# RaghuvirJonnagiri/LatticeBoltzmannSimulations

Hardware: AMD Instinct MI355X
Metric: MLUPS (million lattice updates/sec) D2Q9 MRT cavity (higher is better)
Workload: dtype f32

## Files before the change

### latticeboltzmannsimulations_amd/csrc/lbm_plan.hip

```cpp
#include "lbm_host.hpp"

namespace lbmhost {

bool frame_lds_fits(const Plan& pl, int S, bool deep_rows, int extra, long long budget) {
    if (!pl.frame_lds) return false;
    const int F = pl.tb_f, L = pl.frame_seg, m = S - 1, np = pl.semantics == LBM_SEM_BOUNCE_BACK_SOLID ? Q : pl.nplanes;
    const long long row_strip = (long long)(L + 2 * m + 2) * (F + m + (deep_rows ? m + extra : 0) + 2);
    const long long col_strip = (long long)(F + m + 2) * (L + 2 * m + extra + 2);
    return 2 * np * std::max(row_strip, col_strip) * pl.es <= budget;
}
int pairs_waves(int S) { return std::min(SP_MAX_WAVES, S + 2); }
StreamPlan plan_stream_on(const Plan& pl, int S, int ncu, long long* cost_out) {
    const bool walls = walls_inside(pl);
    const int V = 16 / pl.es, Rr = stream_rim(S, V), TXu = 64 * V - 2 * Rr, F = walls ? 0 : pl.tb_f;
    const int cols = pl.geo.nx - 2 * F;
    const int rows = walls ? pl.geo.ny - pl.tb_f * neighbours(pl) : pl.geo.ny - 2 * F;
    StreamPlan best{walls ? stream_walls_strips(pl.geo.nx, S, V) : (cols + TXu - 1) / TXu, 1, rows};
    long long best_cost = -1;
    for (int n = 1; n <= 256 && n * 8 <= std::max(rows, 8); ++n) {
        const int H = (rows + n - 1) / n, nseg = (rows + H - 1) / H;
        const long long segs = (long long)best.nstrips * nseg, rounds = (segs + ncu - 1) / ncu;
        long long iters = H + 2 * (S - 1) + ST_WAVES - 1;
        if (pl.kern == Kern::stream_pairs) {
            const long long Wv = pairs_waves(S), np = (H + 2 * (S - 1) + 1) / 2;
            iters = 2 * Wv * ((np + Wv - 1) / Wv) + 2 * Wv;
        }
        const long long cost = rounds * iters;
        if (best_cost < 0 || cost < best_cost) { best_cost = cost; best.nsegy = nseg; best.H = H; }
    }
    if (cost_out) *cost_out = best_cost;
    return best;
}
StreamPlan plan_stream(const Plan& pl, int S) {
    long long cost0 = 0;
    const StreamPlan p0 = plan_stream_on(pl, S, pl.ncu, &cost0);
    const bool walls = walls_inside(pl);
    if (!(is_slab(pl) && pl.deep_halo && (pl.frame_fused || walls) && pl.edge_reserve) || S < 3) return p0;
    if ((long long)p0.nstrips * p0.nsegy > pl.ncu) return p0;
    const int nb = neighbours(pl), L = pl.frame_seg;
    const long long n_edge = walls ? (long long)nb * p0.nstrips
                                   : (long long)nb * p0.nstrips + 2LL * frame_segs(pl.geo.ny, L) + (2LL - nb) * frame_segs(pl.geo.nx, L);
    const long long edge_it = pl.tb_f + 2 * (S - 1) + ST_WAVES - 1;
    if (walls ? cost0 > 3 * edge_it : 4 * cost0 > 7 * edge_it) return p0;
    StreamPlan best = p0;
    long long best_cost = cost0 + edge_it * ((n_edge + pl.ncu - 1) / pl.ncu);
    const long long grain = walls ? 32 : 1;
    auto in_grains = [&](long long n) { return (n + grain - 1) / grain * grain; };
    if (walls && in_grains((long long)p0.nstrips * p0.nsegy) + in_grains(n_edge) <= pl.ncu) best_cost = std::max(cost0, edge_it);
    for (int div = 1; div <= (walls ? 1 : 3); ++div) {
        const long long r = in_grains((n_edge + div - 1) / div);
        if (r < 1 || r > pl.ncu / 2) continue;
        long long cb = 0;
        const StreamPlan sp = plan_stream_on(pl, S, pl.ncu - (int)r, &cb);
        const long long cost = std::max(cb, edge_it * ((n_edge + r - 1) / r));
        if (cost < best_cost) { best_cost = cost; best = sp; }
    }
    return best;
}

bool lag_replayable(const Plan& pl, int S) {
    if (S <= 1) return true;
    if (!pl.lazy_lag || pl.push) return false;
    if (!is_slab(pl)) return true;
    return pl.deep_halo && S - 1 >= 3;
}

int unit_steps(const Plan& pl, int left, bool raw, bool own_transport) {
    if (left < 1) return 0;
    if (pl.kern == Kern::none || raw) return 1;
    const int T = pl.tb_steps;
    if (is_slab(pl) && !pl.deep_halo && !own_transport) return 1;
    if (!lag_replayable(pl, T)) {
        if (left >= T + 1) return T;
        if (T >= 3 && left - 1 >= 3) return left - 1;
        return 1;
    }
    if (T == 2) return left >= 2 ? 2 : 1;
    const int m = is_slab(pl) ? 4 : 3;
    if (left >= T) {
        const int r = left - T;
        if (r == 0 || r >= m) return T;
        if (left - m >= m) return left - m;
        return T;
    }
    return left >= m ? left : 1;
}

Route unit_route(const Plan& pl, int S, bool replay) {
    const bool slab = is_slab(pl), deep = slab && pl.deep_halo;
    if (replay && S < 3) return Route::single_steps;
    if (!slab && ((walls_inside(pl) && S >= 2) || (S >= 3 && pl.frame_fused && (replay || !(pl.kern == Kern::stream && pl.frame_beside)))))
        return Route::one_launch;
    if (S >= 3 && deep && streaming(pl) && (pl.frame_fused || walls_inside(pl))) return Route::edges_bulk;
    if (S >= 3 && pl.frame_fused && (!slab || deep)) return Route::fused_frame;
    return Route::frame_passes;
}


std::string validate_params(const lbm_params* p) {
    if (!p || p->struct_size != (int32_t)sizeof(lbm_params)) return std::string("lbm_params.struct_size mismatch");
    if (p->nx < 4 || p->ny < 4) return std::string("nx, ny must be >= 4");
    if (p->y0 < 0 || p->ny_local < 2 || p->y0 + p->ny_local > p->ny) return std::string("slab rows out of range (ny_local >= 2)");
    if (p->ny_local > 65535) return std::string("ny_local > 65535 not supported");
    if (p->dtype != LBM_F32 && p->dtype != LBM_F64) return std::string("dtype must be LBM_F32 or LBM_F64");
    if (p->collision < LBM_SRT || p->collision > LBM_MRT) return std::string("collision must be SRT, TRT or MRT");
    if (p->semantics < LBM_SEM_MRT_PY || p->semantics > LBM_SEM_BOUNCE_BACK_SOLID) return std::string("bad semantics");
    if (p->turb != 0 && p->turb != 1) return std::string("turb must be 0 or 1");
    if (p->turb == 1 && p->semantics != LBM_SEM_MRT_GPU) return std::string("turb = 1 (Smagorinsky, MRT_GPU.py:368-387) exists only with MRT_GPU semantics");
    if (p->kernel < LBM_KERNEL_AUTO || p->kernel > LBM_KERNEL_STREAM) return std::string("bad kernel variant");
    if (p->kernel == LBM_KERNEL_PUSH && (p->turb || p->batch > 1 || p->y0 != 0 || p->ny_local != p->ny))
        return std::string("kernel = PUSH (the reference's two-launch scheme, for A/B) takes one whole lattice without the closure");
    if (p->layout < LBM_LAYOUT_AUTO || p->layout > LBM_LAYOUT_ROWS) return std::string("bad layout");
    if (p->batch < 0 || p->batch > 65535) return std::string("batch must be 0 .. 65535");
    if (p->arith != LBM_ARITH_STRICT && p->arith != LBM_ARITH_FAST && p->arith != LBM_ARITH_PROMOTED)
        return std::string("arith must be LBM_ARITH_STRICT, LBM_ARITH_FAST or LBM_ARITH_PROMOTED");
    if (p->arith == LBM_ARITH_PROMOTED && p->semantics != LBM_SEM_MRT_GPU)
        return std::string("arith = promoted exists only with MRT_GPU semantics (promotion is a property of MRT_GPU.py's CUDA text; "
                           "MRT.py semantics is NumPy fp64)");
    if (p->arith == LBM_ARITH_PROMOTED && (p->flags & LBM_FLAG_STREAM_PAIRS))
        return std::string("arith = promoted does not run on the streaming kernel with two rows per wave (LBM_FLAG_STREAM_PAIRS)");
    if ((p->flags & LBM_FLAG_SOLID_TILES) && p->semantics != LBM_SEM_BOUNCE_BACK_SOLID)
        return std::string("LBM_FLAG_SOLID_TILES (solid obstacles on the multi-step tile kernel) needs a solid mask: semantics = LBM_SEM_BOUNCE_BACK_SOLID");
    if (p->semantics == LBM_SEM_BOUNCE_BACK_SOLID) {
        if (p->y0 != 0 || p->ny_local != p->ny)
            return std::string("solid obstacles (LBM_SEM_BOUNCE_BACK_SOLID) take whole lattices: no slabs (y0 = 0, ny_local = ny)");
        if (p->flags & LBM_FLAG_SOLID_TILES) {
            if (p->kernel != LBM_KERNEL_AUTO && p->kernel != LBM_KERNEL_TB)
                return std::string("LBM_FLAG_SOLID_TILES runs the tile kernel, kernel = AUTO or TB: STREAM / VEC / PUSH have no solid path, GENERIC is "
                                   "one step per launch (leave the flag out)");
            if (p->tb_steps == 2)
                return std::string("LBM_FLAG_SOLID_TILES: tb_steps must be 0 (default) or 3 .. 5 (the two-step tile kernel has no solid path)");
        } else if (p->kernel != LBM_KERNEL_AUTO && p->kernel != LBM_KERNEL_GENERIC)
            return std::string("solid obstacles (LBM_SEM_BOUNCE_BACK_SOLID) step one step per launch, kernel = AUTO or GENERIC: TB / STREAM / VEC / PUSH "
                               "never compute a cell next to a solid one (the tile kernel does with LBM_FLAG_SOLID_TILES)");
    }
    if (p->semantics == LBM_SEM_BOUNCE_BACK || p->semantics == LBM_SEM_BOUNCE_BACK_SOLID) {
        if (p->arith == LBM_ARITH_PROMOTED)
            return std::string("arith = promoted (MRT_GPU.py's CUDA text) does not exist with bounce-back walls (LBM_SEM_BOUNCE_BACK)");
        if (p->kernel == LBM_KERNEL_PUSH || p->kernel == LBM_KERNEL_VEC)
            return std::string("kernel = PUSH / VEC have MRT_GPU.py's wall rules built in: bounce-back walls (LBM_SEM_BOUNCE_BACK) run GENERIC, TB or STREAM");
        if (p->flags & (LBM_FLAG_STREAM_WALLS | LBM_FLAG_STREAM_PAIRS))
            return std::string("LBM_FLAG_STREAM_WALLS / STREAM_PAIRS: the streaming kernels with the walls inside have MRT_GPU.py's wall rules built in, "
                               "bounce-back walls (LBM_SEM_BOUNCE_BACK) run with the wall frame");
    }
    if (p->batch > 1 && (p->y0 != 0 || p->ny_local != p->ny)) return std::string("a batch of lattices cannot be slab-decomposed");
    if (p->ny_local_min < 0 || p->ny_local_min > p->ny_local) return std::string("ny_local_min must be 0 or the smallest ny_local of all ranks (<= ny_local)");
    if (p->tb_steps != 0 && (p->tb_steps < 2 || p->tb_steps > SP_MAX_S)) return std::string("tb_steps must be 0 (default) or 2 .. " + std::to_string(SP_MAX_S));
    if (p->frame_seg != 0 && p->frame_seg < 8) return std::string("frame_seg must be 0 (default) or >= 8");
    if ((p->flags & LBM_FLAG_NT_ON) && (p->flags & LBM_FLAG_NT_OFF)) return std::string("LBM_FLAG_NT_ON and LBM_FLAG_NT_OFF exclude each other");
    return std::string();
}

static int ny_plan(const lbm_params& p) { return p.ny_local_min > 0 ? p.ny_local_min : p.ny_local; }
static bool one_launch(const Plan& pl) { return pl.batch == 1 && !is_slab(pl) && pl.frame_fused; }

struct Forced {
    int nt = 0, frame_beside = 0;
    bool stream_walls = false, stream_pairs = false, no_stream_walls = false, no_tail_tiles = false;
};
static Forced decode_flags(const lbm_params& p, Plan& pl) {
    const auto on = [&](int bit) { return (p.flags & bit) != 0; };
    pl.deep_halo = p.semantics == LBM_SEM_MRT_GPU && !on(LBM_FLAG_NO_DEEP_HALO);
    pl.frame_fused = !on(LBM_FLAG_FRAME_UNFUSED);
    pl.frame_lds = !on(LBM_FLAG_NO_FRAME_LDS);
    pl.frame_wide = !on(LBM_FLAG_FRAME_NARROW);
    pl.lazy_lag = !on(LBM_FLAG_EAGER_LAG);
    pl.xcd_bands = !on(LBM_FLAG_NO_XCD_BANDS);
    pl.edge_first = !on(LBM_FLAG_NO_EDGE_FIRST);
    pl.edge_reserve = !on(LBM_FLAG_NO_EDGE_RESERVE);
    pl.comm_priority = !on(LBM_FLAG_COMM_PRIORITY_OFF);
    Forced f;
    f.nt = on(LBM_FLAG_NT_ON) ? 1 : on(LBM_FLAG_NT_OFF) ? -1 : 0;
    f.frame_beside = on(LBM_FLAG_FRAME_BESIDE_ON) ? 1 : on(LBM_FLAG_FRAME_BESIDE_OFF) ? -1 : 0;
    f.stream_walls = on(LBM_FLAG_STREAM_WALLS);
    f.stream_pairs = on(LBM_FLAG_STREAM_PAIRS);
    f.no_stream_walls = on(LBM_FLAG_NO_STREAM_WALLS);
    f.no_tail_tiles = on(LBM_FLAG_NO_TAIL_TILES);
    pl.solid_tiles = on(LBM_FLAG_SOLID_TILES);
    return f;
}

static void plan_geometry(Plan& pl, const lbm_params& p, const Forced& f) {
    pl.es = p.dtype == LBM_F32 ? 4 : 8;
    pl.geo.nx = p.nx;
    pl.geo.ny = p.ny_local;
    pl.geo.y0 = p.y0;
    pl.geo.NY = p.ny;
    pl.geo.pitch = ((p.nx + 2 * GH) + 3) / 4 * 4;
    pl.nplanes = p.turb ? Q + 2 : Q;
    if (p.semantics == LBM_SEM_BOUNCE_BACK_SOLID) pl.nplanes = Q + 1;
    pl.semantics = p.semantics;
    if (p.layout == LBM_LAYOUT_PLANES) {
        pl.geo.plane = (long long)pl.geo.pitch * (p.ny_local + 2 * GHY);
        pl.geo.row = pl.geo.pitch;
    } else {
        pl.geo.plane = pl.geo.pitch;
        pl.geo.row = (long long)pl.nplanes * pl.geo.pitch;
    }
    pl.batch = p.batch > 1 ? p.batch : 1;
    pl.bstride = (long long)pl.nplanes * pl.geo.pitch * (p.ny_local + 2 * GHY);
    pl.lat_bytes = (size_t)pl.bstride * pl.batch * pl.es;
    pl.use_nt = f.nt ? f.nt > 0 : pl.lat_bytes > ((size_t)192 << 20);
}

static std::string plan_kernel(Plan& pl, const lbm_params& p, const Forced& f, bool device) {
    const int nyp = ny_plan(p), V = 16 / pl.es;
    const bool slab = is_slab(pl);
    if (p.semantics == LBM_SEM_BOUNCE_BACK_SOLID) {
        pl.use_vec = p.nx % V == 0 && p.kernel != LBM_KERNEL_GENERIC;
        pl.kern = Kern::none;
        if (!pl.solid_tiles) return std::string();
        if (p.nx % V != 0 || p.nx < 32 || nyp < 32)
            return "LBM_FLAG_SOLID_TILES needs what kernel = TB needs: nx % (16 / sizeof(real)) == 0, nx >= 32 and ny >= 32";
        pl.kern = Kern::tile;
        return std::string();
    }
    const bool can_vec = p.semantics == LBM_SEM_MRT_GPU && p.nx % V == 0;
    if (p.kernel == LBM_KERNEL_VEC && !can_vec) return "kernel = VEC needs MRT_GPU semantics and nx % (16 / sizeof(real)) == 0";
    pl.push = p.kernel == LBM_KERNEL_PUSH;
    pl.use_vec = can_vec && p.kernel != LBM_KERNEL_GENERIC && !pl.push;
    const bool can_tb = p.nx % V == 0 && p.nx >= 32 && nyp >= 32;
    if (p.kernel == LBM_KERNEL_TB && !can_tb) return "kernel = TB needs nx % (16 / sizeof(real)) == 0, nx >= 32 and ny_local >= 32 (on every rank)";
    const bool big = one_launch(pl) ? (p.nx >= 64 && nyp >= 64) : (long long)p.nx * nyp * pl.batch >= 768LL * 768LL;
    const bool can_stream = can_tb && p.nx >= 64 && nyp >= 64 && pl.batch == 1;
    if (p.kernel == LBM_KERNEL_STREAM && !can_stream)
        return "kernel = STREAM takes one lattice (no batch) with nx % (16 / sizeof(real)) == 0, nx >= 64, ny_local >= 64 (on every rank)";
    const long long cells_plan = (long long)p.nx * nyp;
    const bool walls_variant = pl.batch == 1 && !slab && p.semantics == LBM_SEM_MRT_GPU && !p.turb && !f.no_stream_walls &&
                               (p.collision == LBM_MRT || p.collision == LBM_SRT);
    const bool walls_pays = walls_variant && (pl.es == 8 ? p.nx >= 1024 && cells_plan >= (1LL << 20)
                                                         : (p.nx >= 4096 && cells_plan >= (2LL << 20)) || (p.nx >= 2048 && cells_plan >= (4LL << 20)));
    const bool stream_pays = walls_pays ||
                             (p.nx >= 2048 ? (slab ? cells_plan >= (1LL << 20) && nyp >= 512 : cells_plan >= ((pl.es == 8 ? 4LL : 8LL) << 20))
                                            : cells_plan >= 3072LL * 3072);
    if (!can_stream || !(p.kernel == LBM_KERNEL_STREAM || (p.kernel == LBM_KERNEL_AUTO && stream_pays))) {
        pl.kern = can_tb && (p.kernel == LBM_KERNEL_TB || (p.kernel == LBM_KERNEL_AUTO && big)) ? Kern::tile : Kern::none;
        return std::string();
    }
    const bool forced = f.stream_walls || f.stream_pairs;
    const bool walls_ok = pl.batch == 1 && p.semantics == LBM_SEM_MRT_GPU && (!slab || pl.deep_halo);
    bool walls_pay = !p.turb && (p.collision == LBM_MRT || p.collision == LBM_SRT);
    if (walls_ok && walls_pay && device && !forced) {
        dispatch(p, [&](auto v) {
            using VT = decltype(v);
            using R = typename VT::R;
            if constexpr (VT::SEM == SEM_GPU) {
                hipFuncAttributes at;
                const void* kern = slab ? reinterpret_cast<const void*>(&k_stream_walls_slab<R, VT::COLL, VT::TURB>)
                                        : reinterpret_cast<const void*>(&k_stream_walls<R, VT::COLL, VT::TURB>);
                if (hipFuncGetAttributes(&at, kern) != hipSuccess || at.localSizeBytes > (p.collision == LBM_SRT ? 128u : 64u))
                    walls_pay = false;
            }
        });
    }
    const bool walls = walls_ok && !f.no_stream_walls && (walls_pay || forced);
    pl.kern = !walls ? Kern::stream : !slab && f.stream_pairs ? Kern::stream_pairs : Kern::stream_walls;
    return std::string();
}

static std::string plan_steps(Plan& pl, const lbm_params& p, const Forced& f) {
    const int nyp = ny_plan(p);
    if (streaming(pl)) {
        pl.tb_steps = p.tb_steps ? p.tb_steps : ST_MAX_S;
        const int fmin = p.semantics == LBM_SEM_MRT_PY ? 1 : 0;
        pl.tb_f = (pl.tb_steps + fmin + 3) / 4 * 4;
        while (pl.tb_steps > 2 && (p.nx < 2 * pl.tb_f + 16 || nyp < 2 * pl.tb_f + 16)) {
            pl.tb_steps -= 1;
            pl.tb_f = (pl.tb_steps + fmin + 3) / 4 * 4;
        }
        if (pl.kern == Kern::stream_pairs) pl.tb_steps = p.tb_steps ? p.tb_steps : 10;
        else if (pl.tb_steps > ST_MAX_S)
            return "tb_steps " + std::to_string(ST_MAX_S + 1) + " .. " + std::to_string(SP_MAX_S) + " need the streaming kernel with two rows per wave (a lone lattice, MRT_GPU semantics)";
        if (pl.kern == Kern::stream_walls && is_slab(pl) && pl.tb_steps < 3) pl.kern = Kern::stream;
        pl.tail_tiles = pl.kern == Kern::stream && !is_slab(pl) && pl.es == 4 && p.semantics != LBM_SEM_MRT_PY && !f.no_tail_tiles;
        return std::string();
    }
    const bool trt_turb = p.turb && p.collision == LBM_TRT;
    const bool fast = p.arith == LBM_ARITH_FAST;
    const bool mrt_plain = p.collision == LBM_MRT && !p.turb;
    const int want32 = fast ? (p.collision == LBM_TRT ? 4 : 5) : (trt_turb ? 3 : (mrt_plain ? 5 : 4));
    const int want64 = p.collision == LBM_MRT ? (fast || mrt_plain ? 5 : 3) : 4;
    const bool small_lone = one_launch(pl) && (long long)p.nx * nyp <= 512LL * 512;
    const int want = p.tb_steps ? p.tb_steps : small_lone ? (p.dtype == LBM_F32 ? 5 : std::max(4, want64))
                                                            : (p.dtype == LBM_F32 ? want32 : want64);
    if (want > 5) return "tb_steps 6 .. " + std::to_string(SP_MAX_S) + " need kernel = STREAM (above " + std::to_string(ST_MAX_S) + ": a lone lattice in MRT_GPU semantics)";
    pl.tb_steps = want == 2 ? 2 : ((want == 4 || want == 5) && p.nx >= 64 && nyp >= 64 ? want : 3);
    pl.tb_f = pl.tb_steps >= 4 ? 2 * TB_F : TB_F;
    if (pl.kern == Kern::tile && pl.tb_steps == 2) pl.kern = Kern::tile2;
    return std::string();
}

static void plan_frame(Plan& pl, const lbm_params& p, const Forced& f, bool device) {
    if (pl.kern == Kern::stream && !is_slab(pl) && f.frame_beside > 0) {
        pl.frame_beside = true;
    } else if (pl.kern == Kern::stream && !is_slab(pl) && f.frame_beside == 0 && pl.es == 8 && device) {
        int rs = 1 << 20, rf = 1 << 20;
        dispatch(p, [&](auto v) {
            using VT = decltype(v);
            using R = typename VT::R;
            hipFuncAttributes at;
            if constexpr (sem_multi_step(VT::SEM, true)) {
                if (hipFuncGetAttributes(&at, reinterpret_cast<const void*>(&k_stream<R, VT::COLL, VT::SEM, VT::TURB>)) == hipSuccess) rs = at.numRegs;
                if (hipFuncGetAttributes(&at, reinterpret_cast<const void*>(&k_frame_beside<R, VT::COLL, VT::SEM, VT::TURB>)) == hipSuccess) rf = at.numRegs;
            }
        });
        pl.frame_beside = (rs + 7) / 8 * 8 * 4 + (rf + 7) / 8 * 8 <= 512;
    }
    if ((pl.frame_seg = p.frame_seg)) return;
    const long long cells1 = (long long)p.nx * ny_plan(p) * pl.batch;
    pl.frame_seg = cells1 <= 512LL * 512 ? 16 : (cells1 <= 1024LL * 1024 ? 32 : 64);
    if (pl.kern == Kern::tile && pl.frame_fused && !is_slab(pl) && pl.frame_lds)
        while (pl.frame_seg > 16 && !frame_lds_fits(pl, pl.tb_steps, false, 0, TILE_FRAME_LDS_BYTES)) pl.frame_seg -= 8;
    if (streaming(pl) && pl.frame_lds)
        while (pl.frame_seg > 16 && !frame_lds_fits(pl, pl.tb_steps, false, 1, ST_LDS_BYTES)) pl.frame_seg -= 8;
    if (pl.frame_beside) {
        const long long per = 2LL * p.nx + 2LL * (ny_plan(p) - 2 * pl.tb_f);
        pl.frame_seg = std::max(64, (int)(((per + pl.ncu - 1) / pl.ncu + 7) / 8 * 8));
    }
}

bool make_plan(const lbm_params& p, int ncu, bool device, Plan& pl, std::string& err) {
    pl = Plan{};
    pl.ncu = ncu;
    const Forced f = decode_flags(p, pl);
    plan_geometry(pl, p, f);
    err = plan_kernel(pl, p, f, device);
    if (err.empty()) err = plan_steps(pl, p, f);
    if (!err.empty()) return false;
    plan_frame(pl, p, f, device);
    return true;
}

static int describe_plan(const Plan& pl, int lattices_held, char* buf, size_t len) {
    static const char* const names[] = {"none", "k_step2_deep", "k_stepS_deep", "k_stream", "k_stream_walls", "k_stream_pairs"};
    const int S = pl.kern != Kern::none ? pl.tb_steps : 1;
    long long wgs = 0, wave_updates = 0;
    const int V = 16 / pl.es;
    if (streaming(pl)) {
        const StreamPlan sp = plan_stream(pl, S);
        wgs = (long long)sp.nstrips * sp.nsegy;
        const int nbr = neighbours(pl);
        const long long rows = pl.geo.ny - (walls_inside(pl) ? nbr * pl.tb_f : 2 * pl.tb_f);
        wave_updates = (long long)sp.nstrips * (rows + ((long long)sp.nsegy * 2 - (walls_inside(pl) ? 2 - nbr : 0)) * (S - 1)) * S;
    } else if (pl.kern == Kern::tile) {
        const int F = pl.tb_f, RV = (S - 1 + V - 1) / V, TX = (16 - 2 * RV) * V, TY = 32 - 2 * (S - 1);
// ... 89 lines not shown
```

### latticeboltzmannsimulations_amd/csrc/lbm_stream.hpp

```cpp
#pragma once
#include "lbm_kernels.hpp"

constexpr int ST_WAVES = 16;
constexpr int ST_NT = ST_WAVES * 64;
constexpr int ST_MAX_S = ST_WAVES / 2;
constexpr int ST_LDS_BYTES = ST_WAVES * 9 * 1024;

__device__ __forceinline__ int dpp_from_lower(int v) { return __builtin_amdgcn_update_dpp(v, v, 0x138, 0xf, 0xf, false); }
__device__ __forceinline__ int dpp_from_upper(int v) { return __builtin_amdgcn_update_dpp(v, v, 0x130, 0xf, 0xf, false); }
__device__ __forceinline__ float lane_lower(float v) { return __builtin_bit_cast(float, dpp_from_lower(__builtin_bit_cast(int, v))); }
__device__ __forceinline__ float lane_upper(float v) { return __builtin_bit_cast(float, dpp_from_upper(__builtin_bit_cast(int, v))); }
__device__ __forceinline__ double lane_lower(double v) {
    const long long b = __builtin_bit_cast(long long, v);
    const unsigned lo = (unsigned)dpp_from_lower((int)(unsigned)b), hi = (unsigned)dpp_from_lower((int)(unsigned)(b >> 32));
    return __builtin_bit_cast(double, (long long)(((unsigned long long)hi << 32) | lo));
}
__device__ __forceinline__ double lane_upper(double v) {
    const long long b = __builtin_bit_cast(long long, v);
    const unsigned lo = (unsigned)dpp_from_upper((int)(unsigned)b), hi = (unsigned)dpp_from_upper((int)(unsigned)(b >> 32));
    return __builtin_bit_cast(double, (long long)(((unsigned long long)hi << 32) | lo));
}

__device__ __forceinline__ float lane_lower_e(float v, float edge) {
    return __builtin_bit_cast(float, __builtin_amdgcn_update_dpp(__builtin_bit_cast(int, edge), __builtin_bit_cast(int, v), 0x138, 0xf, 0xf, false));
}
__device__ __forceinline__ float lane_upper_e(float v, float edge) {
    return __builtin_bit_cast(float, __builtin_amdgcn_update_dpp(__builtin_bit_cast(int, edge), __builtin_bit_cast(int, v), 0x130, 0xf, 0xf, false));
}
__device__ __forceinline__ double lane_lower_e(double v, double edge) {
    const long long b = __builtin_bit_cast(long long, v), e = __builtin_bit_cast(long long, edge);
    const unsigned lo = (unsigned)__builtin_amdgcn_update_dpp((int)(unsigned)e, (int)(unsigned)b, 0x138, 0xf, 0xf, false);
    const unsigned hi = (unsigned)__builtin_amdgcn_update_dpp((int)(unsigned)(e >> 32), (int)(unsigned)(b >> 32), 0x138, 0xf, 0xf, false);
    return __builtin_bit_cast(double, (long long)(((unsigned long long)hi << 32) | lo));
}
__device__ __forceinline__ double lane_upper_e(double v, double edge) {
    const long long b = __builtin_bit_cast(long long, v), e = __builtin_bit_cast(long long, edge);
    const unsigned lo = (unsigned)__builtin_amdgcn_update_dpp((int)(unsigned)e, (int)(unsigned)b, 0x130, 0xf, 0xf, false);
    const unsigned hi = (unsigned)__builtin_amdgcn_update_dpp((int)(unsigned)(e >> 32), (int)(unsigned)(b >> 32), 0x130, 0xf, 0xf, false);
    return __builtin_bit_cast(double, (long long)(((unsigned long long)hi << 32) | lo));
}
template <typename R, int V>
__device__ __forceinline__ typename VecT<R, V>::type shift_from_lower_e(typename VecT<R, V>::type own, R edge) {
    typename VecT<R, V>::type r;
    r[0] = lane_lower_e(own[V - 1], edge);
#pragma unroll
    for (int c = 1; c < V; ++c) r[c] = own[c - 1];
    return r;
}
template <typename R, int V>
__device__ __forceinline__ typename VecT<R, V>::type shift_from_upper_e(typename VecT<R, V>::type own, R edge) {
    typename VecT<R, V>::type r;
#pragma unroll
    for (int c = 0; c < V - 1; ++c) r[c] = own[c + 1];
    r[V - 1] = lane_upper_e(own[0], edge);
    return r;
}

template <typename R, int V>
__device__ __forceinline__ typename VecT<R, V>::type shift_from_lower(typename VecT<R, V>::type own) {
    typename VecT<R, V>::type r;
    r[0] = lane_lower(own[V - 1]);
#pragma unroll
    for (int c = 1; c < V; ++c) r[c] = own[c - 1];
    return r;
}
template <typename R, int V>
__device__ __forceinline__ typename VecT<R, V>::type shift_from_upper(typename VecT<R, V>::type own) {
    typename VecT<R, V>::type r;
#pragma unroll
    for (int c = 0; c < V - 1; ++c) r[c] = own[c + 1];
    r[V - 1] = lane_upper(own[0]);
    return r;
}

__host__ __device__ constexpr int stream_rim(int S, int V) { return (S + V - 1) / V * V; }

#ifdef LBM_EXPERIMENT_NO_BARRIER
__device__ __forceinline__ void lds_barrier() { asm volatile("s_waitcnt lgkmcnt(0)" ::: "memory"); }
#else
__device__ __forceinline__ void lds_barrier() { asm volatile("s_waitcnt lgkmcnt(0)\n\ts_barrier" ::: "memory"); }
#endif

template <typename R, int V, bool PROM = false>
__device__ __forceinline__ void wall_row_rules(typename VecT<R, V>::type (&in)[Q], typename VecT<R, V>::type& rw, bool lid, R uLB, bool wl, bool wr,
                                               R& kl, R& kr) {
    typedef typename VecT<R, V>::type T;
    if (lid) {
        const T ux = T(uLB), uy = T((R)0);
        const T cq = (R)1.5 * (ux * ux + uy * uy);
        auto fek = [&](int k) {
            const T cu = cu_of<T>(k, ux, uy);
            if constexpr (PROM) {
                const T rt = rw * weight<R>(k), usqr = ux * ux + uy * uy;
                T fe;
#pragma unroll
                for (int c = 0; c < V; ++c) fe[c] = feq_prom(rt[c], cu[c], usqr[c]);
                return fe;
            } else {
                return (rw * weight<R>(k)) * ((((R)1. + (R)3.0 * cu) + ((R)4.5 * cu) * cu) - cq);
            }
        };
        if (wl) {
            const R g7 = kl;
            in[1][0] = (fek(1)[0] - fek(3)[0]) + in[3][0];
            in[5][0] = (fek(5)[0] - fek(7)[0]) + g7;
            in[8][0] = (fek(8)[0] - fek(6)[0]) + in[6][0];
        }
        if (wr) {
            const R g8 = kr;
            in[3][V - 1] = (-fek(1)[V - 1] + fek(3)[V - 1]) + in[1][V - 1];
            in[6][V - 1] = (-fek(8)[V - 1] + fek(6)[V - 1]) + g8;
            in[7][V - 1] = (-fek(5)[V - 1] + fek(7)[V - 1]) + in[5][V - 1];
        }
        in[4] = (-fek(2) + fek(4)) + in[2];
        in[7] = (-fek(5) + fek(7)) + in[5];
        in[8] = (-fek(6) + fek(8)) + in[6];
        if (wl) kl = in[7][0];
        if (wr) kr = in[8][V - 1];
        rw = ((in[0] + in[1]) + in[3]) + (R)2. * ((in[2] + in[5]) + in[6]);
    } else {
        if (wl) {
            const R g6 = kl;
            in[1][0] = (R)0 + in[3][0];
            in[5][0] = (R)0 + in[7][0];
            in[8][0] = (R)0 + g6;
        }
        if (wr) {
            const R g5 = kr;
            in[3][V - 1] = (R)0 + in[1][V - 1];
            in[6][V - 1] = (R)0 + in[8][V - 1];
            in[7][V - 1] = (R)0 + g5;
        }
        in[2] = (R)0 + in[4];
        in[5] = (R)0 + in[7];
        in[6] = (R)0 + in[8];
        if (wl) kl = in[6][0];
        if (wr) kr = in[5][V - 1];
    }
}

template <typename R, int V, bool WALLS>
__device__ __forceinline__ void build_in(typename VecT<R, V>::type (&in)[Q], typename VecT<R, V>::type o0, typename VecT<R, V>::type o1,
                                         typename VecT<R, V>::type o3, typename VecT<R, V>::type u2, typename VecT<R, V>::type u5,
                                         typename VecT<R, V>::type u6, typename VecT<R, V>::type d4, typename VecT<R, V>::type d7,
                                         typename VecT<R, V>::type d8) {
    in[0] = o0;
    in[2] = u2;
    in[4] = d4;
    if (WALLS) {
        in[1] = shift_from_lower_e<R, V>(o1, (R)0 + o3[1]);
        in[5] = shift_from_lower_e<R, V>(u5, (R)0 + d7[1]);
        in[8] = shift_from_lower_e<R, V>(d8, (R)0 + u6[1]);
        in[3] = shift_from_upper_e<R, V>(o3, (R)0 + o1[V - 2]);
        in[6] = shift_from_upper_e<R, V>(u6, (R)0 + d8[V - 2]);
        in[7] = shift_from_upper_e<R, V>(d7, (R)0 + u5[V - 2]);
    } else {
        in[1] = shift_from_lower<R, V>(o1);
        in[5] = shift_from_lower<R, V>(u5);
        in[8] = shift_from_lower<R, V>(d8);
        in[3] = shift_from_upper<R, V>(o3);
        in[6] = shift_from_upper<R, V>(u6);
        in[7] = shift_from_upper<R, V>(d7);
    }
}

template <typename R, int COLL, bool TURB, bool WALLS = false, bool SLAB = false>
__device__ __forceinline__ void stream_segment(const R* __restrict__ src, R* __restrict__ dst, const Geo& geo, const Relax<R>& w, R* __restrict__ lds,
                                               int S, int xs, int ya, int yb, int xe, int own_lo = 0, int own_hi = 0) {
    constexpr int V = 16 / (int)sizeof(R), ROW = 64 * V;
    typedef typename VecT<R, V>::type T;
    const int wv = __builtin_amdgcn_readfirstlane((int)(threadIdx.x >> 6)), lane = threadIdx.x & 63;
    const int q = ((wv & 7) << 1) | (wv >> 3);
    const int RV = stream_rim(S, V) / V;
    const bool wall_lo = WALLS && (!SLAB || geo.y0 == 0), wall_hi = WALLS && (!SLAB || geo.y0 + geo.ny == geo.NY);
    const int y_first = wall_lo ? max(ya - (S - 1), 0) : ya - (S - 1);
    const int y_end = wall_hi ? min(yb + (S - 1), geo.ny) : yb + (S - 1);
    const int y_lid = wall_lo ? 0 : -(1 << 30), y_bot = wall_hi ? geo.ny - 1 : -(1 << 30);
    const int nb = y_end - y_first;
    const int x0 = xs + lane * V;
    const bool lane_in = x0 < geo.nx;
    const bool lane_out = WALLS ? (x0 >= own_lo && x0 < own_hi) : (lane >= RV && lane < 64 - RV && x0 < xe);
    const bool wl = WALLS && x0 == 0, wr = WALLS && x0 + V == geo.nx;
    const bool side_strip = WALLS && (xs == 0 || xs + ROW >= geo.nx);
    const bool narrow = WALLS && xs + ROW > geo.nx;
    R* const slot_mine = lds + (q * 9) * ROW;
    R* const up_mine = slot_mine + lane * V;
    const R* const up_below = lds + (((q + 1) & (ST_WAVES - 1)) * 9) * ROW + lane * V;
    const R* const down_above = lds + (((q + ST_WAVES - 1) & (ST_WAVES - 1)) * 9 + 3) * ROW + lane * V;

    T in[Q], outv[Q], hq, hr;
#ifdef LBM_EXP_NO_HBM
    auto row_base = [&](const R* p, int k, int y) { return (const char*)(p + ((long long)k * geo.plane + (long long)((y & 63) + GHY) * geo.row)); };
#else
    auto row_base = [&](const R* p, int k, int y) { return (const char*)(p + ((long long)k * geo.plane + (long long)(y + GHY) * geo.row)); };
#endif
    const unsigned lane_off = (unsigned)(GH + x0) * (unsigned)sizeof(R);
    auto cell = [&](const char* base, int dx) {
        unsigned off = lane_off;
        asm volatile("" : "+v"(off));
        return (const R*)(base + (off + (unsigned)(dx * (int)sizeof(R))));
    };
    const unsigned lane_off_ld = WALLS ? (unsigned)(GH + min(x0, max(geo.nx - V, 0))) * (unsigned)sizeof(R) : lane_off;
    auto cell_ld = [&](const char* base, int dx) {
        unsigned off = lane_off_ld;
        asm volatile("" : "+v"(off));
        return (const R*)(base + (off + (unsigned)(dx * (int)sizeof(R))));
    };
    auto load_row = [&](int y, bool exists) {
        if (WALLS) {
            if (exists) {
#pragma unroll
                for (int k = 0; k < Q; ++k) in[k] = vload<R, V, false>(cell_ld(row_base(src, k, y + cyk(k)), -cxk(k)), cxk(k) == 0);
                if (TURB) {
                    hq = vload<R, V, false>(cell_ld(row_base(src, K_QEQ, y), 0), true);
                    hr = vload<R, V, false>(cell_ld(row_base(src, K_RHO, y), 0), true);
                }
            } else {
#pragma unroll
                for (int k = 0; k < Q; ++k) in[k] = T{};
                hq = hr = T{};
            }
            return;
        }
        if (!lane_in || !exists) return;
#pragma unroll
        for (int k = 0; k < Q; ++k) in[k] = vload<R, V, false>(cell(row_base(src, k, y + cyk(k)), -cxk(k)), cxk(k) == 0);
        if (TURB) {
            hq = vload<R, V, false>(cell(row_base(src, K_QEQ, y), 0), true);
            hr = vload<R, V, false>(cell(row_base(src, K_RHO, y), 0), true);
        }
    };
    auto post = [&](int level, bool up, bool down) __attribute__((always_inline)) {
        R* const dn = up_mine + (3 + (level & 1) * 3) * ROW;
        const T p2 = outv[2], p5 = outv[5], p6 = outv[6], p4 = outv[4], p7 = outv[7], p8 = outv[8];
#ifdef LBM_EXP_NO_LDS
        if (geo.nx < 0)
#endif
        if (up) {
            *reinterpret_cast<T*>(up_mine) = p2;
            *reinterpret_cast<T*>(up_mine + ROW) = p5;
            *reinterpret_cast<T*>(up_mine + 2 * ROW) = p6;
        }
#ifdef LBM_EXP_NO_LDS
        if (geo.nx < 0)
#endif
        if (down) {
            *reinterpret_cast<T*>(dn) = p4;
            *reinterpret_cast<T*>(dn + ROW) = p7;
            *reinterpret_cast<T*>(dn + 2 * ROW) = p8;
        }
    };
    auto block = [&](int b, auto wrow_tag) __attribute__((always_inline)) {
        constexpr bool WROW = decltype(wrow_tag)::value;
        const int y = y_first + b;
        const bool wrow = WALLS && WROW, lid = WALLS && WROW && y == 0;
        R* const st = slot_mine + (lid ? 0 : 3 * ROW);
        auto update = [&](bool first) {
            int kind = 0;
            T rw = T{};
            R kl = (R)0, kr = (R)0;
            if (WALLS) {
                if constexpr (WROW) {
                    if (first) {
                        if (lid) rw = vload<R, V, false>(cell_ld(row_base(src, 0, -1), 0), true);
                        kl = lid ? in[7][0] : in[6][0];
                        kr = lid ? in[8][V - 1] : in[5][V - 1];
                    } else {
                        if (lid) rw = *reinterpret_cast<const T*>(st + lane * V);
                        kl = st[ROW + lane];
                        kr = st[2 * ROW + lane];
                    }
                    wall_row_rules<R, V, coll_is_prom(COLL)>(in, rw, lid, w.uLB, wl, wr, kl, kr);
                    kind = lid ? 1 : 2;
                } else if (side_strip && (first || narrow)) {
                    if (wl && first) { in[1][0] = (R)0 + in[3][0]; in[5][0] = (R)0 + in[7][0]; in[8][0] = (R)0 + in[6][0]; }
                    if (wr) { in[3][V - 1] = (R)0 + in[1][V - 1]; in[6][V - 1] = (R)0 + in[8][V - 1]; in[7][V - 1] = (R)0 + in[5][V - 1]; }
                }
            }
#ifdef LBM_EXP_NO_COLLIDE
#pragma unroll
            for (int k = 0; k < Q; ++k) outv[k] = in[k];
#else
            collide_vec<R, COLL, V, TURB>(in, w, outv, hq, hr, wl && kind == 0, wr && kind == 0, kind);
#endif
            if constexpr (WALLS && WROW) {
                if (lid) *reinterpret_cast<T*>(st + lane * V) = rw;
                st[ROW + lane] = kl;
                st[2 * ROW + lane] = kr;
            }
        };
        const bool up = !lid, down = !(wrow && !lid);
        update(true);
        if (S > 1) post(1, up, down);
        lds_barrier();
        lds_barrier();
        for (int l = 1; l < S; ++l) {
            const R* const dn = down_above + (l & 1) * 3 * ROW;
#ifdef LBM_EXP_NO_LDS
            build_in<R, V, WALLS>(in, outv[0], outv[1], outv[3], outv[2], outv[5], outv[6], outv[4], outv[7], outv[8]);
#else
            build_in<R, V, WALLS>(in, outv[0], outv[1], outv[3], *reinterpret_cast<const T*>(up_below), *reinterpret_cast<const T*>(up_below + ROW),
                                  *reinterpret_cast<const T*>(up_below + 2 * ROW), *reinterpret_cast<const T*>(dn), *reinterpret_cast<const T*>(dn + ROW),
                                  *reinterpret_cast<const T*>(dn + 2 * ROW));
#endif
            update(false);
            if (l + 1 < S) {
                post(l + 1, up, down);
                lds_barrier();
                lds_barrier();
            }
        }
        {
            const T hq_done = hq, hr_done = hr;
            T rw_done = T{};
            R kl_done = (R)0, kr_done = (R)0;
            if (WALLS && wrow) {
                if (lid) rw_done = *reinterpret_cast<const T*>(st + lane * V);
                kl_done = st[ROW + lane];
                kr_done = st[2 * ROW + lane];
            }
            if (lane_out && y >= ya && y < yb) {
#pragma unroll
                for (int k = 0; k < Q; ++k) vstore<R, V, false>(const_cast<R*>(cell(row_base(dst, k, y), 0)), outv[k]);
                if (TURB) {
                    vstore<R, V, false>(const_cast<R*>(cell(row_base(dst, K_QEQ, y), 0)), hq_done);
                    vstore<R, V, false>(const_cast<R*>(cell(row_base(dst, K_RHO, y), 0)), hr_done);
                }
                if (WALLS && wrow) {
                    if (lid) {
                        vstore<R, V, false>(const_cast<R*>(cell(row_base(dst, 0, -1), 0)), rw_done);
                        if (wl) *const_cast<R*>(cell(row_base(dst, 7, -1), 1)) = kl_done;
                        if (wr) *const_cast<R*>(cell(row_base(dst, 8, -1), V - 2)) = kr_done;
                    } else {
                        if (wl) *const_cast<R*>(cell(row_base(dst, 6, geo.ny), 1)) = kl_done;
                        if (wr) *const_cast<R*>(cell(row_base(dst, 5, geo.ny), V - 2)) = kr_done;
                    }
                }
            }
            if (S > 1) lds_barrier();
            load_row(y_first + b + ST_WAVES, b + ST_WAVES < nb);
            if (S > 1) lds_barrier();
        }
        for (int i = 2 * S; i < ST_WAVES; ++i) lds_barrier();
    };
#pragma unroll
    for (int k = 0; k < Q; ++k) in[k] = T{};
    hq = T{}; hr = T{};
    for (int i = 0; i < q; ++i) lds_barrier();
    load_row(y_first + q, q < nb);
    for (int b = q; b < nb; b += ST_WAVES) {
        const int y = y_first + b;
        if (WALLS && (SLAB ? (y == y_lid || y == y_bot) : (y == 0 || y == geo.ny - 1))) block(b, std::true_type{});
        else block(b, std::false_type{});
    }
}

template <typename R, int COLL, int SEM, bool TURB>
__global__ __launch_bounds__(ST_NT) void k_stream(const R* __restrict__ src, R* __restrict__ dst, Geo geo, Relax<R> w, int S, int F, int xe, int ye,
                                                  int nstrips, int H, FramePtrs<R> fp, int nframe, int nsegx, int nsegy, int seg, int use_lds,
                                                  int lo, int hi, int bands, int xcd_bands) {
    __shared__ __align__(16) R lds[ST_LDS_BYTES / sizeof(R)];
    if ((int)blockIdx.x < nframe) {
        frame_passes<R, COLL, SEM, TURB, ST_NT>(fp, 0, geo, w, F, S, nsegx, nsegy, lo, hi, (int)blockIdx.x, seg, use_lds ? lds : nullptr, bands);
        return;
    }
    constexpr int V = 16 / (int)sizeof(R);
    int b = blockIdx.x - nframe;
    if (xcd_bands) {
        const int per = ((int)gridDim.x - nframe) >> 3;
        if (b < (per << 3)) b = (b & 7) * per + (b >> 3);
    }
    const int strip = b % nstrips, sy = b / nstrips;
    const int R_ = stream_rim(S, V);
    const int xs = F - R_ + strip * (64 * V - 2 * R_);
    int ya, yb;
    if (bands) {
        const bool top = (bands & 1) && sy == 0;
        if (top) { ya = -(lo > 0 ? lo - 1 : 0); yb = F; }
        else { ya = geo.ny - F; yb = geo.ny + (hi > 0 ? hi - 1 : 0); }
    } else {
        ya = F + sy * H; yb = min(ye, ya + H);
    }
    if (ya >= yb) return;
    stream_segment<R, COLL, TURB>(src, dst, geo, w, lds, S, xs, ya, yb, xe);
}

__host__ __device__ constexpr int stream_walls_strips(int nx, int S, int V) {
    return nx <= 64 * V ? 1 : (nx - 64 * V + (64 * V - 2 * stream_rim(S, V)) - 1) / (64 * V - 2 * stream_rim(S, V)) + 1;
}
template <int V>
__device__ __forceinline__ void walls_strip(const Geo& geo, int S, int strip, int nstrips, int& xs, int& own_lo, int& own_hi) {
    const int R_ = stream_rim(S, V), TXu = 64 * V - 2 * R_;
    xs = min(strip * TXu, max(geo.nx - 64 * V, 0));
    own_lo = strip == 0 ? 0 : strip * TXu + R_;
    own_hi = strip == nstrips - 1 ? geo.nx : (strip + 1) * TXu + R_;
}

template <typename R, int COLL, bool TURB>
__global__ __launch_bounds__(ST_NT) void k_stream_walls(const R* __restrict__ src, R* __restrict__ dst, Geo geo, Relax<R> w, int S, int nstrips, int H,
                                                        int xcd_bands) {
    __shared__ __align__(16) R lds[ST_LDS_BYTES / sizeof(R)];
    constexpr int V = 16 / (int)sizeof(R);
    const int b = xcd_bands ? xcd_band(blockIdx.x, gridDim.x) : (int)blockIdx.x;
    const int strip = b % nstrips, sy = b / nstrips;
    int xs, own_lo, own_hi;
    walls_strip<V>(geo, S, strip, nstrips, xs, own_lo, own_hi);
    const int ya = sy * H, yb = min(geo.ny, ya + H);
    if (ya >= yb) return;
    stream_segment<R, COLL, TURB, true>(src, dst, geo, w, lds, S, xs, ya, yb, 0, own_lo, own_hi);
}
template <typename R, int COLL, bool TURB>
__global__ __launch_bounds__(ST_NT) void k_stream_walls_slab(const R* __restrict__ src, R* __restrict__ dst, Geo geo, Relax<R> w, int S, int nstrips, int H,
                                                             int xcd_bands, int ybeg, int yend, int bands, int lo, int hi, int F) {
    __shared__ __align__(16) R lds[ST_LDS_BYTES / sizeof(R)];
    constexpr int V = 16 / (int)sizeof(R), W = 64 * V;
    int b = blockIdx.x;
    if (xcd_bands) {
        const int per = (int)gridDim.x >> 3;
        if (b < (per << 3)) b = (b & 7) * per + (b >> 3);
    }
    const int strip = b % nstrips, sy = b / nstrips;
    const int R_ = stream_rim(S, V), TXu = W - 2 * R_;
    const int xs = min(strip * TXu, max(geo.nx - W, 0));
    const int own_lo = strip == 0 ? 0 : strip * TXu + R_;
    const int own_hi = strip == nstrips - 1 ? geo.nx : (strip + 1) * TXu + R_;
    int ya, yb;
    if (bands) {
        const bool top = (bands & 1) && sy == 0;
        if (top) { ya = -(lo > 0 ? lo - 1 : 0); yb = F; }
        else { ya = geo.ny - F; yb = geo.ny + (hi > 0 ? hi - 1 : 0); }
    } else {
        ya = ybeg + sy * H; yb = min(yend, ya + H);
    }
    if (ya >= yb) return;
    stream_segment<R, COLL, TURB, true, true>(src, dst, geo, w, lds, S, xs, ya, yb, 0, own_lo, own_hi);
}

constexpr int SP_MAX_WAVES = 12;
constexpr int SP_NT = SP_MAX_WAVES * 64;

constexpr int SP_MAX_S = SP_MAX_WAVES - 2;
constexpr int SP_SLOTS = 12;
constexpr int SP_LDS_BYTES = SP_MAX_WAVES * SP_SLOTS * 1024;

template <typename R, int COLL, bool TURB>
__device__ __forceinline__ void stream_pairs_segment(const R* __restrict__ src, R* __restrict__ dst, const Geo& geo, const Relax<R>& w, R* __restrict__ lds,
                                                     int S, int xs, int ya, int yb, int own_lo, int own_hi) {
    constexpr int V = 16 / (int)sizeof(R), ROW = 64 * V;
    typedef typename VecT<R, V>::type T;
    const int W = (int)(blockDim.x >> 6);
    const int wv = __builtin_amdgcn_readfirstlane((int)(threadIdx.x >> 6)), lane = threadIdx.x & 63;
    const int y_first = max(ya - (S - 1), 0), y_end = min(yb + (S - 1), geo.ny);
    const int nb = y_end - y_first, npairs = (nb + 1) >> 1;
    const int x0 = xs + lane * V;
    const bool lane_out = x0 >= own_lo && x0 < own_hi;
    const bool wl = x0 == 0, wr = x0 + V == geo.nx;
    const bool side_strip = xs == 0 || xs + ROW >= geo.nx;
    const bool narrow = xs + ROW > geo.nx;
    R* const slot_mine = lds + (wv * SP_SLOTS) * ROW;
    R* const post_mine = slot_mine + lane * V;
    const R* const up_below = lds + (((wv + 1 == W ? 0 : wv + 1)) * SP_SLOTS) * ROW + lane * V;
    const R* const down_above = lds + (((wv == 0 ? W - 1 : wv - 1)) * SP_SLOTS + 3) * ROW + lane * V;

    T in[Q], outv[Q], rawB[Q];
    T a0, a1, a3, a4, a7, a8, b0, b1, b3, b2, b5, b6;
    T hqA, hrA, hqB, hrB;
    auto row_base = [&](const R* p, int k, int y) __attribute__((always_inline)) { return (const char*)(p + ((long long)k * geo.plane + (long long)(y + GHY) * geo.row)); };
    const unsigned lane_off = (unsigned)(GH + x0) * (unsigned)sizeof(R);
    auto cell = [&](const char* base, int dx) __attribute__((always_inline)) {
        unsigned off = lane_off;
        asm volatile("" : "+v"(off));
        return (const R*)(base + (off + (unsigned)(dx * (int)sizeof(R))));
    };
    const unsigned lane_off_ld = (unsigned)(GH + min(x0, max(geo.nx - V, 0))) * (unsigned)sizeof(R);
    auto cell_ld = [&](const char* base, int dx) __attribute__((always_inline)) {
        unsigned off = lane_off_ld;
        asm volatile("" : "+v"(off));
        return (const R*)(base + (off + (unsigned)(dx * (int)sizeof(R))));
    };
    auto load_pair = [&](int j) __attribute__((always_inline)) {
        if (j < npairs) {
            const int yA = y_first + 2 * j, yB = yA + 1;
#pragma unroll
            for (int k = 0; k < Q; ++k) in[k] = vload<R, V, false>(cell_ld(row_base(src, k, yA + cyk(k)), -cxk(k)), cxk(k) == 0);
            if (TURB) {
                hqA = vload<R, V, false>(cell_ld(row_base(src, K_QEQ, yA), 0), true);
                hrA = vload<R, V, false>(cell_ld(row_base(src, K_RHO, yA), 0), true);
            }
            const int yBc = min(yB, y_end - 1);
#pragma unroll
            for (int k = 0; k < Q; ++k) rawB[k] = vload<R, V, false>(cell_ld(row_base(src, k, yBc + cyk(k)), -cxk(k)), cxk(k) == 0);
            if (TURB) {
                hqB = vload<R, V, false>(cell_ld(row_base(src, K_QEQ, yBc), 0), true);
                hrB = vload<R, V, false>(cell_ld(row_base(src, K_RHO, yBc), 0), true);
            }
        } else {
#pragma unroll
            for (int k = 0; k < Q; ++k) { in[k] = T{}; rawB[k] = T{}; }
            hqA = hrA = hqB = hrB = T{};
        }
    };
    auto park_B = [&]() __attribute__((always_inline)) {
#pragma unroll
        for (int k = 0; k < Q; ++k) *reinterpret_cast<T*>(post_mine + (3 + k) * ROW) = rawB[k];
    };
    auto update = [&](int y, bool first, T& hq, T& hr, auto wp_tag) __attribute__((always_inline)) {
        constexpr bool WP = decltype(wp_tag)::value;
        int kind = 0;
        if constexpr (WP) {
            const bool wrow = y == 0 || y == geo.ny - 1, lid = y == 0;
            R* const st = slot_mine + (lid ? 0 : 3 * ROW);
            T rw = T{};
            R kl = (R)0, kr = (R)0;
            if (wrow) {
                if (first) {
                    if (lid) rw = vload<R, V, false>(cell_ld(row_base(src, 0, -1), 0), true);
                    kl = lid ? in[7][0] : in[6][0];
                    kr = lid ? in[8][V - 1] : in[5][V - 1];
                } else {
                    if (lid) rw = *reinterpret_cast<const T*>(st + lane * V);
                    kl = st[ROW + lane];
                    kr = st[2 * ROW + lane];
                }
                wall_row_rules<R, V, coll_is_prom(COLL)>(in, rw, lid, w.uLB, wl, wr, kl, kr);
                kind = lid ? 1 : 2;
                if (lid) *reinterpret_cast<T*>(st + lane * V) = rw;
                st[ROW + lane] = kl;
                st[2 * ROW + lane] = kr;
            }
        }
        if (kind == 0 && side_strip && (first || narrow)) {
            if (wl && first) { in[1][0] = (R)0 + in[3][0]; in[5][0] = (R)0 + in[7][0]; in[8][0] = (R)0 + in[6][0]; }
            if (wr) { in[3][V - 1] = (R)0 + in[1][V - 1]; in[6][V - 1] = (R)0 + in[8][V - 1]; in[7][V - 1] = (R)0 + in[5][V - 1]; }
        }
        collide_vec<R, COLL, V, TURB>(in, w, outv, hq, hr, wl && kind == 0, wr && kind == 0, kind);
    };
    auto store_row = [&](int y, const T& hq, const T& hr) __attribute__((always_inline)) {
        if (!(lane_out && y >= ya && y < yb)) return;
#pragma unroll
        for (int k = 0; k < Q; ++k) vstore<R, V, false>(const_cast<R*>(cell(row_base(dst, k, y), 0)), outv[k]);
        if (TURB) {
            vstore<R, V, false>(const_cast<R*>(cell(row_base(dst, K_QEQ, y), 0)), hq);
            vstore<R, V, false>(const_cast<R*>(cell(row_base(dst, K_RHO, y), 0)), hr);
        }
        if (y == 0 || y == geo.ny - 1) {
            const bool lid = y == 0;
            const R* const st = slot_mine + (lid ? 0 : 3 * ROW);
            const R kl = st[ROW + lane], kr = st[2 * ROW + lane];
            if (lid) {
                vstore<R, V, false>(const_cast<R*>(cell(row_base(dst, 0, -1), 0)), *reinterpret_cast<const T*>(st + lane * V));
                if (wl) *const_cast<R*>(cell(row_base(dst, 7, -1), 1)) = kl;
                if (wr) *const_cast<R*>(cell(row_base(dst, 8, -1), V - 2)) = kr;
            } else {
                if (wl) *const_cast<R*>(cell(row_base(dst, 6, geo.ny), 1)) = kl;
                if (wr) *const_cast<R*>(cell(row_base(dst, 5, geo.ny), V - 2)) = kr;
            }
        }
    };
#pragma unroll
    for (int k = 0; k < Q; ++k) { in[k] = T{}; rawB[k] = T{}; }
    hqA = hrA = hqB = hrB = T{};
    a0 = a1 = a3 = a4 = a7 = a8 = b0 = b1 = b3 = b2 = b5 = b6 = T{};
    const int rounds = (npairs + W - 1) / W;
    const int total = 2 * W * rounds + 2 * W;
    int done = 2 * wv;
    load_pair(wv);
    for (int i = 0; i < 2 * wv; ++i) {
        if (i == 2) park_B();
        lds_barrier();
    }
    if (2 * wv <= 2) park_B();
    auto pair_body = [&](int j, auto wp_tag) __attribute__((always_inline)) {
        const int yA = y_first + 2 * j, yB = yA + 1;
        const bool lidA = yA == 0, botB = yB >= geo.ny - 1;
        auto after_A = [&](int l1) __attribute__((always_inline)) {
            a0 = outv[0]; a1 = outv[1]; a3 = outv[3]; a4 = outv[4]; a7 = outv[7]; a8 = outv[8];
            const T p2 = outv[2], p5 = outv[5], p6 = outv[6];
            if (l1 < S) {
                if (!lidA) {
                    *reinterpret_cast<T*>(post_mine) = p2;
                    *reinterpret_cast<T*>(post_mine + ROW) = p5;
                    *reinterpret_cast<T*>(post_mine + 2 * ROW) = p6;
                }
            } else {
                store_row(yA, hqA, hrA);
            }
            lds_barrier();
        };
        auto after_B = [&](int l1) __attribute__((always_inline)) {
            b0 = outv[0]; b1 = outv[1]; b3 = outv[3]; b2 = outv[2]; b5 = outv[5]; b6 = outv[6];
            const T p4 = outv[4], p7 = outv[7], p8 = outv[8];
            if (l1 < S) {
                if (!botB) {
                    R* const dn = post_mine + (3 + (l1 & 1) * 3) * ROW;
                    *reinterpret_cast<T*>(dn) = p4;
                    *reinterpret_cast<T*>(dn + ROW) = p7;
                    *reinterpret_cast<T*>(dn + 2 * ROW) = p8;
                }
            }
            lds_barrier();
        };
        update(yA, true, hqA, hrA, wp_tag);
        after_A(1);
#pragma unroll
        for (int k = 0; k < Q; ++k) in[k] = *reinterpret_cast<const T*>(post_mine + (3 + k) * ROW);
        update(yB, true, hqB, hrB, wp_tag);
        after_B(1);
        for (int l = 1; l < S; ++l) {
            {
                const R* const dn = down_above + (l & 1) * 3 * ROW;
                build_in<R, V, true>(in, a0, a1, a3, b2, b5, b6, *reinterpret_cast<const T*>(dn), *reinterpret_cast<const T*>(dn + ROW),
                                     *reinterpret_cast<const T*>(dn + 2 * ROW));
                *reinterpret_cast<T*>(post_mine + 9 * ROW) = a4;
                *reinterpret_cast<T*>(post_mine + 10 * ROW) = a7;
                *reinterpret_cast<T*>(post_mine + 11 * ROW) = a8;
                update(yA, false, hqA, hrA, wp_tag);
                after_A(l + 1);
            }
            {
                build_in<R, V, true>(in, b0, b1, b3, *reinterpret_cast<const T*>(up_below), *reinterpret_cast<const T*>(up_below + ROW),
                                     *reinterpret_cast<const T*>(up_below + 2 * ROW), *reinterpret_cast<const T*>(post_mine + 9 * ROW),
                                     *reinterpret_cast<const T*>(post_mine + 10 * ROW), *reinterpret_cast<const T*>(post_mine + 11 * ROW));
                update(yB, false, hqB, hrB, wp_tag);
                after_B(l + 1);
            }
        }
        {
            const T hq_done = hqB, hr_done = hrB;
            load_pair(j + W);
            store_row(yB, hq_done, hr_done);
        }
    };
    for (int j = wv; j < npairs; j += W) {
        const int yA = y_first + 2 * j;
        if (yA == 0 || yA + 1 >= geo.ny - 1) pair_body(j, std::true_type{});
        else pair_body(j, std::false_type{});
        for (int i = 2 * S; i < 2 * W; ++i) {
            if (i == 2 * S + 2) park_B();
            lds_barrier();
        }
        done += 2 * W;
    }
    for (; done < total; ++done) lds_barrier();
}

template <typename R, int COLL, bool TURB>
// ... 13 lines not shown
```

Baseline: 377,600.

## Trim stream kernel tail levels and drain barriers, update planner cost model

The temporal-blocked stream kernel now computes fewer time levels for trailing rows past the last owned row, skips the row load and barriers when no further block follows, and shortens the final barrier drain. The slot indexing is factored into a small shared schedule header. The planner's iteration cost now uses the new schedule formula, which can change the strip and segment choices. This removes redundant wave-pipeline work and barriers at segment ends, but the reduced barrier counts risk mismatched barriers between waves.

```diff
diff --git a/latticeboltzmannsimulations_amd/csrc/lbm_plan.hip b/latticeboltzmannsimulations_amd/csrc/lbm_plan.hip
--- a/latticeboltzmannsimulations_amd/csrc/lbm_plan.hip
+++ b/latticeboltzmannsimulations_amd/csrc/lbm_plan.hip
@@ -10,6 +10,7 @@
     return 2 * np * std::max(row_strip, col_strip) * pl.es <= budget;
 }
 int pairs_waves(int S) { return std::min(SP_MAX_WAVES, S + 2); }
+static long long stream_price_drain(int S) { return ST_WAVES - S; }
 StreamPlan plan_stream_on(const Plan& pl, int S, int ncu, long long* cost_out) {
     const bool walls = walls_inside(pl);
     const int V = 16 / pl.es, Rr = stream_rim(S, V), TXu = 64 * V - 2 * Rr, F = walls ? 0 : pl.tb_f;
@@ -20,7 +21,7 @@
     for (int n = 1; n <= 256 && n * 8 <= std::max(rows, 8); ++n) {
         const int H = (rows + n - 1) / n, nseg = (rows + H - 1) / H;
         const long long segs = (long long)best.nstrips * nseg, rounds = (segs + ncu - 1) / ncu;
-        long long iters = H + 2 * (S - 1) + ST_WAVES - 1;
+        long long iters = stream_iterations(S, S - 1 + H - 1) + stream_price_drain(S);
         if (pl.kern == Kern::stream_pairs) {
             const long long Wv = pairs_waves(S), np = (H + 2 * (S - 1) + 1) / 2;
             iters = 2 * Wv * ((np + Wv - 1) / Wv) + 2 * Wv;
@@ -40,7 +41,7 @@
     const int nb = neighbours(pl), L = pl.frame_seg;
     const long long n_edge = walls ? (long long)nb * p0.nstrips
                                    : (long long)nb * p0.nstrips + 2LL * frame_segs(pl.geo.ny, L) + (2LL - nb) * frame_segs(pl.geo.nx, L);
-    const long long edge_it = pl.tb_f + 2 * (S - 1) + ST_WAVES - 1;
+    const long long edge_it = stream_iterations(S, S - 1 + pl.tb_f - 1) + stream_price_drain(S);
     if (walls ? cost0 > 3 * edge_it : 4 * cost0 > 7 * edge_it) return p0;
     StreamPlan best = p0;
     long long best_cost = cost0 + edge_it * ((n_edge + pl.ncu - 1) / pl.ncu);
diff --git a/latticeboltzmannsimulations_amd/csrc/lbm_stream.hpp b/latticeboltzmannsimulations_amd/csrc/lbm_stream.hpp
--- a/latticeboltzmannsimulations_amd/csrc/lbm_stream.hpp
+++ b/latticeboltzmannsimulations_amd/csrc/lbm_stream.hpp
@@ -74,6 +74,8 @@
 }
 
 __host__ __device__ constexpr int stream_rim(int S, int V) { return (S + V - 1) / V * V; }
+
+#include "lbm_stream_sched.hpp"
 
 #ifdef LBM_EXPERIMENT_NO_BARRIER
 __device__ __forceinline__ void lds_barrier() { asm volatile("s_waitcnt lgkmcnt(0)" ::: "memory"); }
@@ -183,10 +185,10 @@
     const bool wl = WALLS && x0 == 0, wr = WALLS && x0 + V == geo.nx;
     const bool side_strip = WALLS && (xs == 0 || xs + ROW >= geo.nx);
     const bool narrow = WALLS && xs + ROW > geo.nx;
-    R* const slot_mine = lds + (q * 9) * ROW;
+    R* const slot_mine = lds + stream_up_slot(q) * ROW;
     R* const up_mine = slot_mine + lane * V;
-    const R* const up_below = lds + (((q + 1) & (ST_WAVES - 1)) * 9) * ROW + lane * V;
-    const R* const down_above = lds + (((q + ST_WAVES - 1) & (ST_WAVES - 1)) * 9 + 3) * ROW + lane * V;
+    const R* const up_below = lds + stream_up_slot((q + 1) & (ST_WAVES - 1)) * ROW + lane * V;
+    const R* const down_above = lds + stream_down_slot((q + ST_WAVES - 1) & (ST_WAVES - 1), 0) * ROW + lane * V;
 
     T in[Q], outv[Q], hq, hr;
 #ifdef LBM_EXP_NO_HBM
@@ -231,7 +233,7 @@
         }
     };
     auto post = [&](int level, bool up, bool down) __attribute__((always_inline)) {
-        R* const dn = up_mine + (3 + (level & 1) * 3) * ROW;
+        R* const dn = up_mine + (stream_down_slot(q, level) - stream_up_slot(q)) * ROW;
         const T p2 = outv[2], p5 = outv[5], p6 = outv[6], p4 = outv[4], p7 = outv[7], p8 = outv[8];
 #ifdef LBM_EXP_NO_LDS
         if (geo.nx < 0)
@@ -290,12 +292,14 @@
             }
         };
         const bool up = !lid, down = !(wrow && !lid);
+        const int n = stream_levels(S, b, yb - 1 - y_first), np = y >= yb ? n + 1 : n;
+        const bool more = b + ST_WAVES < nb;
         update(true);
-        if (S > 1) post(1, up, down);
+        if (np > 1) post(1, up, down);
         lds_barrier();
         lds_barrier();
-        for (int l = 1; l < S; ++l) {
-            const R* const dn = down_above + (l & 1) * 3 * ROW;
+        for (int l = 1; l < n; ++l) {
+            const R* const dn = down_above + (stream_down_slot(0, l) - stream_down_slot(0, 0)) * ROW;
 #ifdef LBM_EXP_NO_LDS
             build_in<R, V, WALLS>(in, outv[0], outv[1], outv[3], outv[2], outv[5], outv[6], outv[4], outv[7], outv[8]);
 #else
@@ -304,7 +308,7 @@
                                   *reinterpret_cast<const T*>(dn + 2 * ROW));
 #endif
             update(false);
-            if (l + 1 < S) {
+            if (l + 1 < np) {
                 post(l + 1, up, down);
                 lds_barrier();
                 lds_barrier();
@@ -337,11 +341,11 @@
                     }
                 }
             }
-            if (S > 1) lds_barrier();
-            load_row(y_first + b + ST_WAVES, b + ST_WAVES < nb);
-            if (S > 1) lds_barrier();
-        }
-        for (int i = 2 * S; i < ST_WAVES; ++i) lds_barrier();
+            if (S > 1 && more) lds_barrier();
+            load_row(y_first + b + ST_WAVES, more);
+            if (S > 1 && more) lds_barrier();
+        }
+        for (int i = more ? 2 * S : ST_WAVES; i < ST_WAVES; ++i) lds_barrier();
     };
 #pragma unroll
     for (int k = 0; k < Q; ++k) in[k] = T{};
diff --git a/latticeboltzmannsimulations_amd/csrc/lbm_stream_sched.hpp b/latticeboltzmannsimulations_amd/csrc/lbm_stream_sched.hpp
--- /dev/null
+++ b/latticeboltzmannsimulations_amd/csrc/lbm_stream_sched.hpp
@@ -0,0 +1,17 @@
+#pragma once
+#if !defined(__HIPCC__) && !defined(__host__)
+#define __host__
+#define __device__
+#endif
+
+__host__ __device__ constexpr int stream_levels(int S, int b, int bL) { return b > bL ? S - (b - bL) : S; }
+__host__ __device__ constexpr int stream_update_it(int b, int l) { return b + 2 * l; }
+__host__ __device__ constexpr int stream_up_slot(int q) { return q * 9; }
+__host__ __device__ constexpr int stream_down_slot(int q, int level) { return q * 9 + 3 + (level & 1) * 3; }
+__host__ __device__ constexpr bool stream_posts(int S, int b, int bL, int level) {
+    return level < stream_levels(S, b, bL) || (b > bL && level == stream_levels(S, b, bL));
+}
+__host__ __device__ constexpr int stream_block_barriers(int S, int b, int nb, int bL, int waves) {
+    return b > bL ? 2 * stream_levels(S, b, bL) : b + waves >= nb ? (S > 1 ? 2 * (S - 1) : 2) : waves;
+}
+__host__ __device__ constexpr int stream_iterations(int S, int bL) { return S > 1 ? bL + 2 * S - 1 : bL + 3; }
```

Result: no change. 374,700 (-0.8%).
